# befelix/safe_learning

Measured on NVIDIA H100. Metric: grid-point Lyapunov checks/sec (2D pendulum, M=500 GP), higher is better.
Workload: dtype f64

## Files before the change

### safe_learning_b200/_build.py

```python

from __future__ import annotations

import os
import subprocess
import sys
from concurrent.futures import ThreadPoolExecutor

HERE = os.path.dirname(os.path.abspath(__file__))
CSRC = os.path.join(HERE, "csrc")
OBJDIR = os.path.join(CSRC, "build")
OUTPUT = os.path.join(HERE, "libslb200.so")
HEADER = os.path.join(HERE, "..", "include", "slb200.h")

UNITS = [("gp_tile_%d_%d.o" % (d, tp), "gp_tile_inst.cu", ["-DSLB_TILE_DIN=%d" % d, "-DSLB_TP=%d" % tp],
          ["gp_tile.cuh", "gp_args.h"]) for d in range(1, 7) for tp in (64, 32)]
UNITS += [("gp_sweep.o", "gp_sweep.cu", [], ["gp_args.h"]),
          ("filter.o", "filter.cu", [], ["bulk_copy.cuh", "exp2_tab512.cuh", "gp_mean_staged.cuh", "gp_mean_grid.cuh",
                                         "gp_args.h"]),
          ("light.o", "light.cu", [], ["bulk_copy.cuh", "exp2_tab512.cuh", "gp_mean_staged.cuh", "bellman.cuh"]),
          ("bellman_tile.o", "bellman_tile.cu", [], []),
          ("rollout.o", "rollout.cu", [], ["bulk_copy.cuh", "exp2_tab512.cuh", "gp_mean_staged.cuh", "bellman.cuh"]),
          ("value_opt.o", "value_opt.cu", [], ["bulk_copy.cuh", "exp2_tab512.cuh", "gp_mean_staged.cuh",
                                               "bellman.cuh"]),
          ("network_grad.o", "network_grad.cu", [], []),
          ("triangulation_grad.o", "triangulation_grad.cu", [], []),
          ("gp_grad.o", "gp_grad.cu", [], []),
          ("gp_hyper.o", "gp_hyper.cu", [], []),
          ("no_shrink.o", "no_shrink.cu", [], [])]
SOURCES = sorted({u[1] for u in UNITS})

ARCH = ["-gencode", "arch=compute_90a,code=sm_90a"]
CFLAGS = ARCH + ["-lineinfo", "-O3", "-std=c++17", "-Xcompiler", "-fPIC"]


def _mtime(path):
    return os.path.getmtime(path) if os.path.exists(path) else 0.0


def _unit_stale(unit):
    obj, src, _, headers = unit
    built = _mtime(os.path.join(OBJDIR, obj))
    deps = [os.path.join(CSRC, src), os.path.join(CSRC, "common.cuh"), os.path.join(CSRC, "exp2_tab64.h"),
            HEADER, os.path.abspath(__file__)]
    deps += [os.path.join(CSRC, h) for h in headers]
    return built == 0.0 or any(_mtime(d) > built for d in deps)


def _stale():
    if not os.path.exists(OUTPUT):
        return True
    built = os.path.getmtime(OUTPUT)
    return any(_unit_stale(u) or _mtime(os.path.join(OBJDIR, u[0])) > built for u in UNITS)


def _run(cmd, verbose):
    proc = subprocess.run(cmd, cwd=CSRC, stdout=subprocess.PIPE, stderr=subprocess.STDOUT, text=True)
    if verbose or proc.returncode != 0:
        sys.stderr.write(proc.stdout)
    if proc.returncode != 0:
        raise RuntimeError("nvcc failed (%s):\n%s" % (" ".join(cmd), proc.stdout))
    return proc.stdout


def build_library(force=False, verbose=False, jobs=None):
    if not force and not _stale():
        return OUTPUT
    nvcc = os.environ.get("NVCC", "nvcc")
    os.makedirs(OBJDIR, exist_ok=True)
    todo = [u for u in UNITS if force or _unit_stale(u)]
    extra = ["-Xptxas", "-v"] if verbose else []

    def compile_unit(unit):
        obj, src, flags, _ = unit
        return _run([nvcc] + CFLAGS + extra + flags + ["-c", src, "-o", os.path.join(OBJDIR, obj)],
                    verbose)

    jobs = jobs or min(len(todo) or 1, os.cpu_count() or 1)
    with ThreadPoolExecutor(max_workers=jobs) as pool:
        list(pool.map(compile_unit, todo))
    _run([nvcc, "-shared"] + ARCH + ["-o", OUTPUT] + [os.path.join(OBJDIR, u[0]) for u in UNITS],
         verbose)
    return OUTPUT


if __name__ == "__main__":
    print(build_library(force="--force" in sys.argv, verbose="-v" in sys.argv))
```

### safe_learning_b200/csrc/gp_args.h

```cpp
#pragma once
#include <stdint.h>

enum { MODE_SWEEP_GRID = 0, MODE_SWEEP_STATES = 1, MODE_PREDICT = 2 };
enum { SLB_SPLIT_ITEMS = 512, SLB_SPLIT_MAX = 8, SLB_SPLIT_TICKET_BYTES = 2048 };
#define SLB_SPLIT_PARTIAL_BYTES ((size_t)SLB_SPLIT_ITEMS * SLB_MAX_OUT * (1 + SLB_MAX_OUT) * 64 * sizeof(double))

struct slb_gp_args {
    const double* points;
    int64_t n;
    int64_t idx_begin;
    int32_t mode;
    int32_t want_var;
    uint8_t* negative;
    double* values;
    double* decrease;
    double* threshold;
    double* mean;
    double* err;
    const int64_t* index_list;
    const unsigned long long* count;
    int64_t count_min, count_max;
    double* split_partial;
    int* split_ticket;
    long long* timing;
};

template <int DIN, int TPV>
int slb_gp_tile_launch(cudaStream_t st, const slb_sweep& cfg, const slb_gp_args& a, bool kexpr, bool timing);
```

### safe_learning_b200/csrc/gp_sweep.cu

```cuda
#include "common.cuh"

#include <string.h>

#include "gp_args.h"

namespace {

__global__ void pack_factor_kernel(const double* __restrict__ Linv, int M, int nrb,
                                   double* __restrict__ W, int64_t total) {
    const int64_t e = (int64_t)blockIdx.x * blockDim.x + threadIdx.x;
    if (e >= total) return;
    const int64_t pair = e >> 6;
    const int lane = (int)((e >> 1) & 31);
    const int half = (int)(e & 1);
    int64_t b = (int64_t)((sqrt(8.0 * (double)pair + 1.0) - 1.0) * 0.5);
    while (b * (b + 1) / 2 > pair) --b;
    while ((b + 1) * (b + 2) / 2 <= pair) ++b;
    const int64_t kp = pair - b * (b + 1) / 2;
    const int64_t row = 8 * b + (lane >> 2);
    const int64_t col = 8 * kp + 4 * half + (lane & 3);
    W[e] = (row < M && col <= row) ? Linv[row * M + col] : 0.0;
}


cudaEvent_t g_factor_event[64] = {};
bool g_factor_pending[64] = {};

int wait_for_factors(cudaStream_t st) {
    int device = 0;
    SLB_CUDA(cudaGetDevice(&device));
    if (device < 0 || device >= 64 || !g_factor_pending[device]) return 0;
    cudaStreamCaptureStatus cs = cudaStreamCaptureStatusNone;
    SLB_CUDA(cudaStreamIsCapturing(st, &cs));
    SLB_CUDA(cudaStreamWaitEvent(st, g_factor_event[device],
                                 cs == cudaStreamCaptureStatusActive ? cudaEventWaitExternal : 0));
    return 0;
}

int dispatch_gp_tile(cudaStream_t st, const slb_sweep& cfg, const slb_gp_args& a, int tp = 64) {
    if (a.n <= 0) return 0;
    if (wait_for_factors(st)) return 1;
    SLB_CHECK(a.n <= (int64_t)0x7fffffff * tp, "too many points for one launch");
    const bool timing = a.timing != nullptr;
    bool kexpr = false;
    for (int f = 0; f < cfg.gp.num_factors; ++f) kexpr |= cfg.gp.factors[f].kernel.num_prims > 0;
    return slb_dispatch_dim<1, 6>(cfg.gp.input_dim, "GP input_dim", [&](auto D) {
        return tp == 64 ? slb_gp_tile_launch<D, 64>(st, cfg, a, kexpr, timing)
                        : slb_gp_tile_launch<D, 32>(st, cfg, a, kexpr, timing);
    });
}

}

int slb_wait_for_factors(cudaStream_t st) { return wait_for_factors(st); }

int slb_launch_det_sweep(cudaStream_t st, const slb_sweep& cfg, const double* states, int64_t n,
                         int64_t idx_begin, uint8_t* negative, double* values, double* decrease,
                         double* threshold, double* mean);

static long long* g_timing_buffer = nullptr;

static int64_t g_refine_split = 32 * SLB_NUM_SMS;

int slb_launch_refine(cudaStream_t st, const slb_sweep& cfg, int64_t n_max, int64_t idx_begin,
                      const int64_t* list, const unsigned long long* count, uint8_t* negative,
                      double* values, double* mean, double* err, double* split_partial, int* split_ticket) {
    slb_gp_args a;
    memset(&a, 0, sizeof(a));
    a.idx_begin = idx_begin; a.mode = MODE_SWEEP_GRID;
    a.negative = negative; a.values = values;
    a.mean = mean; a.err = err;
    a.index_list = list; a.count = count;
    a.timing = g_timing_buffer;
    const int tps[2] = {32, 64};
    const int64_t lo[2] = {0, g_refine_split};
    const int64_t hi[2] = {g_refine_split, INT64_MAX};
    for (int v = 0; v < 2; ++v) {
        if (lo[v] >= hi[v] || lo[v] >= n_max) continue;
        a.count_min = lo[v]; a.count_max = hi[v];
        a.n = n_max < hi[v] ? n_max : hi[v];
        a.split_partial = nullptr; a.split_ticket = nullptr;
        if (v == 0 && split_partial != nullptr) {
            if (a.n < (int64_t)SLB_NUM_SMS * tps[v]) a.n = (int64_t)SLB_NUM_SMS * tps[v];
            if ((a.n + tps[v] - 1) / tps[v] <= SLB_SPLIT_ITEMS) {
                a.split_partial = split_partial; a.split_ticket = split_ticket;
            }
        }
        const int rc = dispatch_gp_tile(st, cfg, a, tps[v]);
        if (rc) return rc;
    }
    return 0;
}

extern "C" {

int slb_debug_refine_split(int64_t upto32) {
    g_refine_split = upto32 < 0 ? 0 : upto32;
    return 0;
}

int slb_restore_tables(void* dst_dev, const void* src_host, int64_t split_bytes, int64_t total_bytes,
                       void* stream, void* side_stream) {
    SLB_CHECK(dst_dev != nullptr && src_host != nullptr, "slb_restore_tables: null buffer");
    SLB_CHECK(split_bytes >= 0 && split_bytes <= total_bytes, "slb_restore_tables: split %lld outside [0, %lld]",
              (long long)split_bytes, (long long)total_bytes);
    cudaStream_t st = static_cast<cudaStream_t>(stream), side = static_cast<cudaStream_t>(side_stream);
    char* dst = static_cast<char*>(dst_dev);
    const char* src = static_cast<const char*>(src_host);
    if (split_bytes > 0) SLB_CUDA(cudaMemcpyAsync(dst, src, (size_t)split_bytes, cudaMemcpyHostToDevice, st));
    const int64_t rest = total_bytes - split_bytes;
    if (rest <= 0) return 0;
    if (side == nullptr || side == st) {
        SLB_CUDA(cudaMemcpyAsync(dst + split_bytes, src + split_bytes, (size_t)rest, cudaMemcpyHostToDevice, st));
        return 0;
    }
    int device = 0;
    SLB_CUDA(cudaGetDevice(&device));
    SLB_CHECK(device >= 0 && device < 64, "slb_restore_tables: device %d unsupported", device);
    static cudaEvent_t order[64] = {};
    if (order[device] == nullptr) SLB_CUDA(cudaEventCreateWithFlags(&order[device], cudaEventDisableTiming));
    SLB_CUDA(cudaEventRecord(order[device], st));
    SLB_CUDA(cudaStreamWaitEvent(side, order[device], 0));
    SLB_CUDA(cudaMemcpyAsync(dst + split_bytes, src + split_bytes, (size_t)rest, cudaMemcpyHostToDevice, side));
    return slb_record_factor_dependency(side);
}

int slb_record_factor_dependency(void* stream) {
    int device = 0;
    SLB_CUDA(cudaGetDevice(&device));
    SLB_CHECK(device >= 0 && device < 64, "slb_record_factor_dependency: device %d unsupported", device);
    if (g_factor_event[device] == nullptr)
        SLB_CUDA(cudaEventCreateWithFlags(&g_factor_event[device], cudaEventDisableTiming));
    SLB_CUDA(cudaEventRecord(g_factor_event[device], static_cast<cudaStream_t>(stream)));
    g_factor_pending[device] = true;
    return 0;
}

int slb_debug_phase_timing(void* buffer_dev) {
    g_timing_buffer = static_cast<long long*>(buffer_dev);
    return 0;
}

int64_t slb_packed_len(int32_t M) {
    if (M <= 0) return 0;
    const int64_t nrb = (M + 7) / 8;
    return nrb * (nrb + 1) * 32;
}

int slb_pack_factor(void* stream, const double* Linv_dev, int32_t M, double* Wpack_dev) {
    SLB_CHECK(Linv_dev != nullptr && Wpack_dev != nullptr, "slb_pack_factor: null pointer");
    SLB_CHECK(M > 0, "slb_pack_factor: M must be positive (got %d)", M);
    const int nrb = (M + 7) / 8;
    const int64_t total = slb_packed_len(M);
    const int threads = 256;
    const int64_t blocks = (total + threads - 1) / threads;
    pack_factor_kernel<<<(unsigned)blocks, threads, 0, (cudaStream_t)stream>>>(Linv_dev, M, nrb,
                                                                              Wpack_dev, total);
    SLB_LAUNCH_CHECK();
    return 0;
}

int slb_gp_predict(void* stream, const slb_gp_stack* gp, const double* points_dev, int64_t n,
                   double* mean_dev, double* err_dev, int32_t want_var) {
    SLB_CHECK(gp != nullptr, "slb_gp_predict: null gp");
    if (slb_validate_gp(gp)) return 1;
    SLB_CHECK(gp->num_outputs > 0, "slb_gp_predict: GP stack has no outputs");
    SLB_CHECK(n >= 0, "slb_gp_predict: negative n");
    SLB_CHECK(n == 0 || (points_dev && mean_dev && err_dev), "slb_gp_predict: null buffer");
    slb_sweep cfg;
    memset(&cfg, 0, sizeof(cfg));
    cfg.gp = *gp;
    slb_gp_args a;
    memset(&a, 0, sizeof(a));
    a.points = points_dev; a.n = n; a.mode = MODE_PREDICT; a.want_var = want_var;
    a.mean = mean_dev; a.err = err_dev;
    return dispatch_gp_tile((cudaStream_t)stream, cfg, a);
}

static int sweep_common(void* stream, const slb_sweep* cfg, const double* states, int64_t n,
                        int64_t idx_begin, uint8_t* negative, double* values, double* decrease,
                        double* threshold, double* mean, double* err) {
    int m;
    if (slb_validate_sweep(cfg, states != nullptr, &m)) return 1;
    SLB_CHECK(n >= 0, "lyapunov sweep: negative point count");
    if (n == 0) return 0;
    SLB_CHECK(negative != nullptr, "lyapunov sweep: negative_dev is required");
    if (cfg->gp.num_outputs > 0) {
        slb_gp_args a;
        memset(&a, 0, sizeof(a));
        a.points = states; a.n = n; a.idx_begin = idx_begin;
        a.mode = states ? MODE_SWEEP_STATES : MODE_SWEEP_GRID;
        a.negative = negative; a.values = values; a.decrease = decrease; a.threshold = threshold;
        a.mean = mean; a.err = err;
        a.timing = g_timing_buffer;
        return dispatch_gp_tile((cudaStream_t)stream, *cfg, a);
    }
    SLB_CHECK(err == nullptr, "deterministic dynamics have no error bounds (err_dev must be NULL)");
    return slb_launch_det_sweep((cudaStream_t)stream, *cfg, states, n, idx_begin, negative, values,
                                decrease, threshold, mean);
}

int slb_lyapunov_sweep(void* stream, const slb_sweep* cfg, int64_t idx_begin, int64_t idx_end,
                       uint8_t* negative_dev, double* values_dev, double* decrease_dev,
                       double* threshold_dev, double* mean_dev, double* err_dev) {
    SLB_CHECK(cfg != nullptr, "slb_lyapunov_sweep: null config");
    if (slb_validate_range("slb_lyapunov_sweep", idx_begin, idx_end, cfg->grid.nindex)) return 1;
    return sweep_common(stream, cfg, nullptr, idx_end - idx_begin, idx_begin, negative_dev,
                        values_dev, decrease_dev, threshold_dev, mean_dev, err_dev);
}

int slb_lyapunov_points(void* stream, const slb_sweep* cfg, const double* states_dev, int64_t n,
                        uint8_t* negative_dev, double* values_dev, double* decrease_dev,
                        double* threshold_dev, double* mean_dev, double* err_dev) {
    SLB_CHECK(n == 0 || states_dev != nullptr, "slb_lyapunov_points: null states");
    return sweep_common(stream, cfg, states_dev, n, 0, negative_dev, values_dev, decrease_dev,
                        threshold_dev, mean_dev, err_dev);
}

}
```

### safe_learning_b200/csrc/gp_tile.cuh

```cuda
#pragma once
#define SLB_EVAL_NOINLINE 1
#include "common.cuh"

#include <string.h>

#include <atomic>


#include "gp_args.h"

namespace {

#ifndef SLB_TP
#define SLB_TP SLB_TILE_POINTS
#endif
constexpr int TP = SLB_TP;
static_assert(TP == 32 || TP == 64, "TP must be 32 or 64");
constexpr int PANEL = 256;
constexpr int KSTR = TP + 2;
constexpr int NW = 8;
constexpr int NT = NW * 32;
constexpr int RQ = 32 / NW;
constexpr int NB = TP / 8;
constexpr int CTAS_PER_SM = 1;
constexpr int NRED = 1 + SLB_MAX_OUT;
constexpr int PREFETCH_CTAS = SLB_NUM_SMS * CTAS_PER_SM;

constexpr size_t SMEM_KS = (size_t)(PANEL / 8) * 4 * KSTR * 2 * sizeof(double);
constexpr size_t SMEM_Z = (size_t)SLB_MAX_IN * TP * sizeof(double);
constexpr size_t SMEM_RED = (size_t)NW * TP * NRED * sizeof(double);
constexpr size_t SMEM_TOT = (size_t)NRED * TP * sizeof(double);
constexpr size_t SMEM_POST = (size_t)2 * SLB_MAX_OUT * TP * sizeof(double);
constexpr size_t SMEM_EXPTAB = 64 * sizeof(double);
constexpr size_t SMEM_XP = (size_t)PANEL * SLB_MAX_IN * sizeof(double);
constexpr size_t SMEM_KEXPR = (sizeof(slb_kernel) + 15) / 16 * 16;
constexpr size_t SMEM_PRE = (size_t)4 * TP * sizeof(double);
constexpr size_t SMEM_TOTAL = SMEM_KS + SMEM_Z + SMEM_RED + SMEM_TOT + SMEM_POST + SMEM_EXPTAB +
                              SMEM_XP + SMEM_KEXPR + SMEM_PRE;

SLB_DEV double2 ldg_stream2(const double2* p) {
    double2 v;
    asm volatile("ld.global.nc.L1::no_allocate.v2.f64 {%0, %1}, [%2];"
                 : "=d"(v.x), "=d"(v.y) : "l"(p));
    return v;
}

SLB_DEV void dmma884(double& c0, double& c1, double a, double b) {
    asm volatile("mma.sync.aligned.m8n8k4.row.col.f64.f64.f64.f64 {%0,%1}, {%2}, {%3}, {%0,%1};"
                 : "+d"(c0), "+d"(c1) : "d"(a), "d"(b));
}

constexpr int RING = TP == 64 ? 3 : 5;
constexpr int BG = 4;

template <int Q0>
SLB_DEV void mma_run(double (&acc)[RQ][NB][2], const double2* const (&ap)[RQ], int m0, int m1,
                     const double2* ks_lane) {
    double2 ar[RING][RQ];
    const int m1m = m1 - 1;
#pragma unroll
    for (int d = 0; d < RING; ++d) {
        const int md = min(m0 + d, m1m);
#pragma unroll
        for (int q = Q0; q < RQ; ++q) ar[d][q] = ldg_stream2(ap[q] + md * 32);
    }
    int m = m0;
#pragma unroll 1
    while (true) {
#pragma unroll
        for (int d = 0; d < RING; ++d) {
            if (m >= m1) return;
            const double2* kb = ks_lane + m * (4 * KSTR);
#pragma unroll
            for (int half = 0; half < NB; half += BG) {
                double2 b[BG];
#pragma unroll
                for (int nb = 0; nb < BG; ++nb) b[nb] = kb[(half + nb) * 8];
#pragma unroll
                for (int q = Q0; q < RQ; ++q)
#pragma unroll
                    for (int nb = 0; nb < BG; ++nb)
                        dmma884(acc[q][half + nb][0], acc[q][half + nb][1], ar[d][q].x, b[nb].x);
#pragma unroll
                for (int q = Q0; q < RQ; ++q)
#pragma unroll
                    for (int nb = 0; nb < BG; ++nb)
                        dmma884(acc[q][half + nb][0], acc[q][half + nb][1], ar[d][q].y, b[nb].y);
            }
            const int mp = min(m + RING, m1m);
#pragma unroll
            for (int q = Q0; q < RQ; ++q) ar[d][q] = ldg_stream2(ap[q] + mp * 32);
            ++m;
        }
    }
}

template <int NBT>
SLB_DEV void row_lane_reduce(const double (&v)[2 * NBT], int lane, double* red_q) {
    constexpr int NV = 2 * NBT;
    const bool g2 = (lane & 16) != 0, g1 = (lane & 8) != 0, g0 = (lane & 4) != 0;
    double w8[NV / 2], w4[NV / 4];
#pragma unroll
    for (int i = 0; i < NV / 2; ++i) {
        const double send = g2 ? v[i] : v[i + NV / 2];
        const double keep = g2 ? v[i + NV / 2] : v[i];
        w8[i] = keep + __shfl_xor_sync(0xffffffffu, send, 16);
    }
#pragma unroll
    for (int i = 0; i < NV / 4; ++i) {
        const double send = g1 ? w8[i] : w8[i + NV / 4];
        const double keep = g1 ? w8[i + NV / 4] : w8[i];
        w4[i] = keep + __shfl_xor_sync(0xffffffffu, send, 8);
    }
    if constexpr (NBT == 8) {
        double w2[2];
#pragma unroll
        for (int i = 0; i < 2; ++i) {
            const double send = g0 ? w4[i] : w4[i + 2];
            const double keep = g0 ? w4[i + 2] : w4[i];
            w2[i] = keep + __shfl_xor_sync(0xffffffffu, send, 4);
        }
        double* slot = red_q + (8 * (lane >> 2) + 2 * (lane & 3)) * NRED;
        slot[0] += w2[0];
        slot[NRED] += w2[1];
    } else {
        static_assert(NBT == 4, "written for 8 or 4 column blocks");
        const double send = g0 ? w4[0] : w4[1];
        const double keep = g0 ? w4[1] : w4[0];
        const double w1 = keep + __shfl_xor_sync(0xffffffffu, send, 4);
        const int g = lane >> 2;
        red_q[(8 * (g >> 1) + 2 * (lane & 3) + (g & 1)) * NRED] += w1;
    }
}

template <int DIN, bool TIMING, bool KEXPR>
SLB_DEV void gp_tile_body(const slb_sweep& cfg, const slb_gp_args& a, unsigned char* smem_raw,
                          const int64_t tile_index, const int64_t npts, const int grp, const int G,
                          const int fsel, const int FS, const bool first_tile) {
    double* Ks = reinterpret_cast<double*>(smem_raw);
    double* zraw = Ks + (PANEL / 8) * 4 * KSTR * 2;
    double* red = zraw + SLB_MAX_IN * TP;
    double* tot = red + NW * TP * NRED;
    double* post = tot + NRED * TP;
    double* exptab = post + 2 * SLB_MAX_OUT * TP;
    double* Xp = exptab + 64;
    slb_kernel* kexpr = reinterpret_cast<slb_kernel*>(Xp + PANEL * SLB_MAX_IN);
    double* pre = reinterpret_cast<double*>(reinterpret_cast<unsigned char*>(kexpr) + SMEM_KEXPR);

    const int tid = threadIdx.x, lane = tid & 31, warp = tid >> 5;
    prefetch_descriptor_operands(cfg);
    const double exp_entry = c_exp2_tab[tid & 63];
    const int64_t tile0 = tile_index * TP;
    const int D = cfg.gp.num_outputs;
    long long t_gen = 0, t_mma = 0, t_epi = 0, t_mark = 0, t_sync = 0, t_s0 = 0;
    const long long t_start = TIMING ? clock64() : 0;
    long long g_start = 0;
    if (TIMING) asm volatile("mov.u64 %0, %globaltimer;" : "=l"(g_start));

    if (first_tile && blockIdx.x < PREFETCH_CTAS) {
        for (int f = 0; f < cfg.gp.num_factors; ++f) {
            const slb_gp_factor& F = cfg.gp.factors[f];
            const char* base = reinterpret_cast<const char*>(F.Wpack);
            const size_t nbytes = (size_t)F.nrb * (F.nrb + 1) * 32 * sizeof(double);
            for (size_t off = ((size_t)blockIdx.x * NT + tid) * 128; off < nbytes;
                 off += (size_t)PREFETCH_CTAS * NT * 128)
                asm volatile("prefetch.global.L2 [%0];" ::"l"(base + off));
        }
    }

    if (tid < 64) exptab[tid] = exp_entry;

    if (tid < TP) {
        int64_t rel = tile0 + tid;
        if (rel > npts - 1) rel = npts - 1;
        if (a.index_list != nullptr) rel = a.index_list[rel];
        double z[SLB_MAX_IN];
        if (a.mode == MODE_PREDICT) {
#pragma unroll
            for (int c = 0; c < DIN; ++c) z[c] = a.points[rel * DIN + c];
        } else {
            const int d = cfg.grid.ndim;
            double x[SLB_MAX_DIM];
            if (a.mode == MODE_SWEEP_GRID) {
                grid_index_to_state(cfg.grid, a.idx_begin + rel, x);
            } else {
                for (int c = 0; c < d; ++c) x[c] = a.points[rel * d + c];
            }
            double u[SLB_MAX_OUT];
            const int m = eval_fn_small(cfg.policy, x, u);
            for (int c = 0; c < d; ++c) z[c] = x[c];
            for (int c = 0; c < m; ++c) z[d + c] = u[c];
        }
#pragma unroll
        for (int c = 0; c < DIN; ++c) zraw[c * TP + tid] = z[c];
    } else if (tid < 2 * TP && a.mode != MODE_PREDICT) {
        const int p = tid - TP;
        int64_t rel = tile0 + p;
        if (rel > npts - 1) rel = npts - 1;
        if (a.index_list != nullptr) rel = a.index_list[rel];
        const int d = cfg.grid.ndim;
        double x[SLB_MAX_DIM];
        if (a.mode == MODE_SWEEP_GRID) {
            grid_index_to_state(cfg.grid, a.idx_begin + rel, x);
        } else {
            for (int c = 0; c < d; ++c) x[c] = a.points[rel * d + c];
        }
        lyapunov_state_terms(cfg, x, a.mode == MODE_SWEEP_GRID ? a.idx_begin + rel : -1, &pre[p],
                             &pre[TP + p]);
    }
    __syncthreads();

    const int wg_ = warp & 3, wr_ = warp >> 2;
    const int wslot = wr_ == 0 ? wg_ : 7 - wg_;
    const int p_gen = tid & (TP - 1);
    const int jg = tid / TP;
    const double2* ks_lane = reinterpret_cast<const double2*>(Ks) + (lane & 3) * KSTR + (lane >> 2);

    auto factor_epilogue = [&](int f, bool general, double s2) {
        const slb_gp_factor& F = cfg.gp.factors[f];
        if (tid < TP) {
            int qty = 1;
            for (int o = 0; o < D; ++o) {
                const slb_gp_output& Go = cfg.gp.outputs[o];
                if (Go.factor != f) continue;
                double mx = 0.0;
                if (Go.prior_mean != nullptr) {
                    mx = f64mul(zraw[tid], Go.prior_mean[0]);
                    for (int c = 1; c < DIN; ++c)
                        mx = f64add(mx, f64mul(zraw[c * TP + tid], Go.prior_mean[c]));
                    mx = f64mul(F.scale, mx);
                }
                const double fmean = f64add(tot[qty * TP + tid], mx) / F.scale;
                double kss = F.kss;
                if (general) {
                    double zt[DIN];
#pragma unroll
                    for (int c = 0; c < DIN; ++c) zt[c] = zraw[c * TP + tid];
                    kss = s2 * kernel_expr_diag<DIN>(*kexpr, zt);
                }
                const double fvar = f64sub(kss, tot[tid]) / s2;
                post[o * TP + tid] = fmean;
                post[(SLB_MAX_OUT + o) * TP + tid] =
                    a.want_var ? fvar : f64mul(Go.beta, sqrt(fvar));
                ++qty;
            }
        }
    };

    const bool split = G * FS > 1;
    for (int f = 0; f < cfg.gp.num_factors; ++f) {
        if (fsel >= 0 && f != fsel) continue;
        const slb_gp_factor& F = cfg.gp.factors[f];
        const int M = F.M, nrb = F.nrb;
        const int nk4 = (M + 3) >> 2;
        const double s2 = f64mul(F.scale, F.scale);
        const double variance = F.variance;
        const double* __restrict__ Xs = F.Xs;

        const bool general = KEXPR && F.kernel.num_prims > 0;
        if (general) {
            __syncthreads();
            const int* src = reinterpret_cast<const int*>(&F.kernel);
            for (int i = tid; i < (int)(sizeof(slb_kernel) / sizeof(int)); i += NT)
                reinterpret_cast<int*>(kexpr)[i] = src[i];
            __syncthreads();
        }
        double zs[DIN];
#pragma unroll
        for (int c = 0; c < DIN; ++c)
            zs[c] = general ? zraw[c * TP + p_gen] : zraw[c * TP + p_gen] / F.lengthscales[c];
        for (int i = lane; i < TP * NRED; i += 32) red[warp * TP * NRED + i] = 0.0;
        __syncwarp();
        int resident = -1;

        int rlo = 0, rhi = nrb;
        if (G > 1) {
            rlo = __double2int_rd((double)nrb * sqrt((double)grp / (double)G));
            rhi = grp + 1 == G ? nrb : __double2int_rd((double)nrb * sqrt((double)(grp + 1) / (double)G));
        }
        for (int pbeg = rlo; pbeg < rhi; pbeg += 32) {
            double acc[RQ][NB][2];
#pragma unroll
            for (int q = 0; q < RQ; ++q)
#pragma unroll
                for (int nb = 0; nb < NB; ++nb) { acc[q][nb][0] = 0.0; acc[q][nb][1] = 0.0; }

            const int pend = min(pbeg + 32, rhi);
            int bq[RQ];
#pragma unroll
            for (int q = 0; q < RQ; ++q) bq[q] = pend - 1 - wslot - NW * (RQ - 1 - q);

            const int jp_last = (pend - 1) >> 5;
            for (int jp = 0; jp <= jp_last; ++jp) {
                const int nkp = min(64, nk4 - 64 * jp);
                if (jp != resident) {
                    if (TIMING) t_s0 = clock64();
                    __syncthreads();
                    if (TIMING) { t_mark = clock64(); t_sync += t_mark - t_s0; }
                    const int j0 = PANEL * jp;
                    const int nj = min(PANEL, M - j0);
                    for (int i = tid; i < nj * DIN; i += NT) Xp[i] = Xs[(size_t)j0 * DIN + i];
                    __syncthreads();
                    constexpr int PS = NT / TP / 4;
                    static_assert(NT / TP == 4 * PS, "generation needs a multiple of 4 groups");
                    const int gr = jg & 3, gpo = jg >> 2;
                    const int npairs = (nkp + 1) >> 1;
                    double2* ks2 = reinterpret_cast<double2*>(Ks);
                    constexpr int GP = 2;
                    if (general) {
                        for (int mm = gpo; mm < npairs; mm += GP * PS) {
                            const double* xr[2 * GP];
#pragma unroll
                            for (int u = 0; u < 2 * GP; ++u) {
                                const int jj = 8 * (mm + PS * (u >> 1)) + 4 * (u & 1) + gr;
                                xr[u] = Xp + min(jj, nj - 1) * DIN;
                            }
                            double kv[2 * GP];
                            kernel_expr_cross_n<DIN, 2 * GP>(*kexpr, zs, xr, exptab, kv);
#pragma unroll
                            for (int u = 0; u < 2 * GP; ++u) {
                                const int jj = 8 * (mm + PS * (u >> 1)) + 4 * (u & 1) + gr;
                                kv[u] = jj < nj ? s2 * kv[u] : 0.0;
                            }
#pragma unroll
                            for (int g = 0; g < GP; ++g)
                                if (mm + PS * g < npairs)
                                    ks2[((mm + PS * g) * 4 + gr) * KSTR + p_gen] =
                                        make_double2(kv[2 * g], kv[2 * g + 1]);
                        }
                    } else
                    for (int mm = gpo; mm < npairs; mm += GP * PS) {
                        double t2[2 * GP];
#pragma unroll
                        for (int u = 0; u < 2 * GP; ++u) {
                            const int jj = min(8 * (mm + PS * (u >> 1)) + 4 * (u & 1) + gr, nj - 1);
                            const double* xr = Xp + jj * DIN;
                            double acc2 = 0.0;
#pragma unroll
                            for (int c = 0; c < DIN; ++c) {
                                const double df = zs[c] - xr[c];
                                acc2 = fma(df, df, acc2);
                            }
                            t2[u] = acc2;
                        }
                        double kv[2 * GP];
#pragma unroll
                        for (int u = 0; u < 2 * GP; ++u) {
                            const int jj = 8 * (mm + PS * (u >> 1)) + 4 * (u & 1) + gr;
                            const double k = s2 * (variance * exp_neg_tab(-0.5 * t2[u], exptab));
                            kv[u] = jj < nj ? k : 0.0;
                        }
#pragma unroll
                        for (int g = 0; g < GP; ++g)
                            if (mm + PS * g < npairs)
                                ks2[((mm + PS * g) * 4 + gr) * KSTR + p_gen] =
                                    make_double2(kv[2 * g], kv[2 * g + 1]);
                    }
                    resident = jp;
                    if (TIMING) { t_s0 = clock64(); t_gen += t_s0 - t_mark; }
                    __syncthreads();
                    if (TIMING) t_sync += clock64() - t_s0;
                }
                if (TIMING) t_mark = clock64();
                const int npairs_mma = (nkp + 1) >> 1;
                int mend[RQ];
                const double2* ap[RQ];
#pragma unroll
                for (int q = 0; q < RQ; ++q) {
                    const bool valid = bq[q] >= pbeg;
                    const int me = valid ? min(npairs_mma, max(0, bq[q] - 32 * jp + 1)) : 0;
                    mend[q] = me;
                    const int64_t b = valid ? bq[q] : 0;
                    ap[q] = reinterpret_cast<const double2*>(F.Wpack) +
                            (b * (b + 1) / 2 + 32 * jp) * 32 + lane;
                }
                int mprev = 0;
                if (mend[0] > mprev) { mma_run<0>(acc, ap, mprev, mend[0], ks_lane); mprev = mend[0]; }
                if (mend[1] > mprev) { mma_run<1>(acc, ap, mprev, mend[1], ks_lane); mprev = mend[1]; }
                if (mend[2] > mprev) { mma_run<2>(acc, ap, mprev, mend[2], ks_lane); mprev = mend[2]; }
                if (mend[3] > mprev) { mma_run<3>(acc, ap, mprev, mend[3], ks_lane); mprev = mend[3]; }
                if (TIMING) t_mma += clock64() - t_mark;
            }
            if (TIMING) t_mark = clock64();

            int qty = 0;
            for (int o = -1; o < D; ++o) {
                double al[RQ] = {};
                if (o >= 0) {
                    if (cfg.gp.outputs[o].factor != f) continue;
                    const double* alpha = cfg.gp.outputs[o].alpha;
#pragma unroll
                    for (int q = 0; q < RQ; ++q)
                        if (bq[q] >= pbeg) al[q] = __ldg(alpha + 8 * bq[q] + (lane >> 2));
                }
                constexpr int NV = 2 * NB;
                double v[NV];
#pragma unroll
                for (int nb = 0; nb < NB; ++nb) {
#pragma unroll
                    for (int e = 0; e < 2; ++e) {
                        double t = 0.0;
#pragma unroll
                        for (int q = 0; q < RQ; ++q) {
                            const double x = acc[q][nb][e];
                            t = fma(x, (o < 0) ? x : al[q], t);
                        }
                        v[nb * 2 + e] = t;
                    }
                }
                row_lane_reduce<NB>(v, lane, red + (size_t)warp * TP * NRED + qty);
                ++qty;
            }
            __syncwarp();
            if (TIMING) t_epi += clock64() - t_mark;
        }

        if (TIMING) t_s0 = clock64();
        __syncthreads();
        if (TIMING) t_sync += clock64() - t_s0;
        if (tid < TP) {
            for (int r = 0; r < NRED; ++r) {
                double s = 0.0;
#pragma unroll
                for (int w = 0; w < NW; ++w) s += red[(w * TP + tid) * NRED + r];
                tot[r * TP + tid] = s;
            }
        }
        __syncthreads();

        if (split) {
            double* part = a.split_partial + ((size_t)blockIdx.x * SLB_MAX_OUT + f) * (NRED * TP);
            for (int i = tid; i < NRED * TP; i += NT) part[i] = tot[i];
            __syncthreads();
            continue;
        }
        factor_epilogue(f, general, s2);
        __syncthreads();
    }

    if (split) {
        __shared__ int s_ticket;
        __threadfence();
        __syncthreads();
        if (tid == 0) s_ticket = atomicAdd(a.split_ticket + tile_index, 1);
        __syncthreads();
        if (s_ticket != G * FS - 1) {
            if (TIMING && lane == 0) {
                long long* t = a.timing + ((size_t)blockIdx.x * NW + warp) * 8;
                long long g_end;
                asm volatile("mov.u64 %0, %globaltimer;" : "=l"(g_end));
                t[0] = t_gen; t[1] = t_mma; t[2] = t_epi; t[3] = clock64() - t_start;
                t[4] = g_start; t[5] = g_end; t[6] = t_sync; t[7] = 1;
            }
            return;
        }
        __threadfence();
        if (tid == 0) a.split_ticket[tile_index] = 0;
        for (int f = 0; f < cfg.gp.num_factors; ++f) {
            const slb_gp_factor& F = cfg.gp.factors[f];
            for (int i = tid; i < NRED * TP; i += NT) {
                double sum = 0.0;
                const size_t cta0 = (size_t)tile_index * (G * FS) + (FS > 1 ? (size_t)f * G : 0);
                for (int g2 = 0; g2 < G; ++g2)
                    sum += __ldcg(a.split_partial + ((cta0 + g2) * SLB_MAX_OUT + f) * (NRED * TP) + i);
                tot[i] = sum;
            }
            const bool general = KEXPR && F.kernel.num_prims > 0;
            if (general) {
                const int* src = reinterpret_cast<const int*>(&F.kernel);
                for (int i = tid; i < (int)(sizeof(slb_kernel) / sizeof(int)); i += NT)
                    reinterpret_cast<int*>(kexpr)[i] = src[i];
            }
            __syncthreads();
            factor_epilogue(f, general, f64mul(F.scale, F.scale));
            __syncthreads();
        }
    }

    if (TIMING && lane == 0) {
        long long* t = a.timing + ((size_t)blockIdx.x * NW + warp) * 8;
        long long g_end;
        asm volatile("mov.u64 %0, %globaltimer;" : "=l"(g_end));
        t[0] = t_gen; t[1] = t_mma; t[2] = t_epi; t[3] = clock64() - t_start;
        t[4] = g_start; t[5] = g_end; t[6] = t_sync; t[7] = 0;
    }
    {
        const int p = tid & (TP - 1);
        const bool live = tile0 + p < npts;
        int64_t rel = live ? tile0 + p : 0;
        if (a.index_list != nullptr) rel = a.index_list[rel];
        if (tid < 2 * TP && live) {
            double mu[SLB_MAX_OUT], er[SLB_MAX_OUT];
            for (int o = 0; o < D; ++o) {
                mu[o] = post[o * TP + p];
                er[o] = post[(SLB_MAX_OUT + o) * TP + p];
            }
            if (tid < TP) {
                if (a.mean != nullptr) for (int o = 0; o < D; ++o) a.mean[rel * D + o] = mu[o];
                if (a.err != nullptr) for (int o = 0; o < D; ++o) a.err[rel * D + o] = er[o];
                if (a.mode != MODE_PREDICT) {
                    double vm[1];
                    eval_fn_small(cfg.lyapunov, mu, vm);
                    pre[2 * TP + p] = vm[0];
                }
            } else if (a.mode != MODE_PREDICT) {
                pre[3 * TP + p] = lyapunov_error_bound(cfg, mu, er);
            }
        }
        if (a.mode == MODE_PREDICT) return;
        __syncthreads();
        if (tid < TP && live) {
            const slb_decision r =
                lyapunov_combine(pre[p], pre[TP + p], pre[2 * TP + p], pre[3 * TP + p]);
            a.negative[rel] = r.negative ? 1 : 0;
            if (a.values != nullptr) a.values[rel] = r.vx;
            if (a.decrease != nullptr) a.decrease[rel] = r.decrease;
            if (a.threshold != nullptr) a.threshold[rel] = r.threshold;
        }
    }
}

template <int DIN, bool TIMING, bool KEXPR, int TPV>
__global__ void __launch_bounds__(NT, CTAS_PER_SM)
gp_tile_kernel(const __grid_constant__ slb_sweep cfg, const slb_gp_args a) {
    extern __shared__ __align__(16) unsigned char smem_raw[];
    int64_t tile_index = blockIdx.x;
    int64_t tile_end = tile_index + 1, tile_step = 1;
    int grp = 0, G = 1;
    int fsel = -1, FS = 1;
    int64_t npts = a.n;
    if (a.count != nullptr) {
        prefetch_descriptor_operands(cfg);
        npts = (int64_t)*a.count;
        if (npts <= a.count_min || npts > a.count_max) return;
        const int64_t ntiles = (npts + TP - 1) / TP;
        if (a.split_partial != nullptr) {
            int64_t spare = (int64_t)gridDim.x / ntiles;
            const int nfac = cfg.gp.num_factors;
            if (nfac > 1 && spare >= 2 * nfac) {
                FS = nfac;
                spare /= nfac;
            }
            G = (int)(spare < 1 ? 1 : (spare > SLB_SPLIT_MAX ? SLB_SPLIT_MAX : spare));
            const int per_tile = G * FS;
            if ((int64_t)blockIdx.x >= ntiles * per_tile) return;
            tile_index = blockIdx.x / per_tile;
            tile_end = tile_index + 1;
            const int rem = (int)(blockIdx.x % per_tile);
            grp = rem % G;
            if (FS > 1) fsel = rem / G;
        } else {
            tile_end = ntiles;
            tile_step = gridDim.x;
        }
        if (tile_index * TP >= npts) return;
    }
    for (int64_t tile = tile_index; tile < tile_end; tile += tile_step) {
        gp_tile_body<DIN, TIMING, KEXPR>(cfg, a, smem_raw, tile, npts, grp, G, fsel, FS, tile == tile_index);
        if (tile + tile_step < tile_end) __syncthreads();
    }
}

template <int DIN, bool TIMING, bool KEXPR, int TPV = TP>
int launch_gp_tile(cudaStream_t st, const slb_sweep& cfg, const slb_gp_args& a) {
    static_assert(TPV == TP, "TPV only disambiguates the symbol");
    static std::atomic<bool> configured[64];
    int device = 0;
    SLB_CUDA(cudaGetDevice(&device));
    if (device < 0 || device >= 64 || !configured[device].load(std::memory_order_acquire)) {
        SLB_CUDA(cudaFuncSetAttribute(gp_tile_kernel<DIN, TIMING, KEXPR, TP>,
                                      cudaFuncAttributeMaxDynamicSharedMemorySize,
                                      (int)SMEM_TOTAL));
        if (device >= 0 && device < 64) configured[device].store(true, std::memory_order_release);
    }
    int64_t tiles = (a.n + TP - 1) / TP;
    if (a.count != nullptr && a.split_partial == nullptr && tiles > PREFETCH_CTAS) tiles = PREFETCH_CTAS;
    gp_tile_kernel<DIN, TIMING, KEXPR, TP><<<(unsigned)tiles, NT, SMEM_TOTAL, st>>>(cfg, a);
    SLB_LAUNCH_CHECK();
    return 0;
}

}
```

### safe_learning_b200/csrc/gp_tile_inst.cu

```cuda
#include "gp_tile.cuh"

#ifndef SLB_TILE_DIN
#error "compile with -DSLB_TILE_DIN=<1..6>"
#endif

template <int DIN, int TPV>
int slb_gp_tile_launch(cudaStream_t st, const slb_sweep& cfg, const slb_gp_args& a, bool kexpr,
                       bool timing) {
#if SLB_TILE_DIN == 3 && SLB_TP == 64
    if (timing) return launch_gp_tile<3, true, false>(st, cfg, a);
#else
    if (timing) {
        slb_set_error("phase timing is compiled for d_in = 3, 64-point tiles only");
        return 1;
    }
#endif
    return kexpr ? launch_gp_tile<DIN, false, true>(st, cfg, a)
                 : launch_gp_tile<DIN, false, false>(st, cfg, a);
}

template int slb_gp_tile_launch<SLB_TILE_DIN, SLB_TP>(cudaStream_t, const slb_sweep&, const slb_gp_args&,
                                                      bool, bool);
```

Before: 546.9 million.

## Merge two refine launches into one kernel choosing tile size on device

The refine path used to launch two GP tile kernels, a 32-point variant and a 64-point variant, each gated by count ranges. Now one refine kernel reads the device-side count and branches between the 32-point split path and the 64-point persistent path, with the long path in a noinline function. This removes one kernel launch per refine and the empty launch that used to exit early. The sweep kernel is simplified to a plain per-tile launch, and the timing instrumentation is extended. The change adds register pressure and code-size risk from putting both tile sizes in one kernel.

```diff
diff --git a/safe_learning_b200/_build.py b/safe_learning_b200/_build.py
--- a/safe_learning_b200/_build.py
+++ b/safe_learning_b200/_build.py
@@ -12,8 +12,8 @@
 OUTPUT = os.path.join(HERE, "libslb200.so")
 HEADER = os.path.join(HERE, "..", "include", "slb200.h")
 
-UNITS = [("gp_tile_%d_%d.o" % (d, tp), "gp_tile_inst.cu", ["-DSLB_TILE_DIN=%d" % d, "-DSLB_TP=%d" % tp],
-          ["gp_tile.cuh", "gp_args.h"]) for d in range(1, 7) for tp in (64, 32)]
+UNITS = [("gp_%s_%d.o" % (kind, d), "gp_tile_inst.cu", ["-DSLB_TILE_DIN=%d" % d, "-DSLB_REFINE=%d" % refine],
+          ["gp_tile.cuh", "gp_args.h"]) for d in range(1, 7) for kind, refine in (("tile", 0), ("refine", 1))]
 UNITS += [("gp_sweep.o", "gp_sweep.cu", [], ["gp_args.h"]),
           ("filter.o", "filter.cu", [], ["bulk_copy.cuh", "exp2_tab512.cuh", "gp_mean_staged.cuh", "gp_mean_grid.cuh",
                                          "gp_args.h"]),
diff --git a/safe_learning_b200/csrc/gp_args.h b/safe_learning_b200/csrc/gp_args.h
--- a/safe_learning_b200/csrc/gp_args.h
+++ b/safe_learning_b200/csrc/gp_args.h
@@ -19,11 +19,13 @@
     double* err;
     const int64_t* index_list;
     const unsigned long long* count;
-    int64_t count_min, count_max;
+    int64_t split_max;
     double* split_partial;
     int* split_ticket;
     long long* timing;
 };
 
-template <int DIN, int TPV>
+template <int DIN>
 int slb_gp_tile_launch(cudaStream_t st, const slb_sweep& cfg, const slb_gp_args& a, bool kexpr, bool timing);
+template <int DIN>
+int slb_gp_refine_launch(cudaStream_t st, const slb_sweep& cfg, const slb_gp_args& a, bool kexpr, bool timing);
diff --git a/safe_learning_b200/csrc/gp_sweep.cu b/safe_learning_b200/csrc/gp_sweep.cu
--- a/safe_learning_b200/csrc/gp_sweep.cu
+++ b/safe_learning_b200/csrc/gp_sweep.cu
@@ -37,16 +37,16 @@
     return 0;
 }
 
-int dispatch_gp_tile(cudaStream_t st, const slb_sweep& cfg, const slb_gp_args& a, int tp = 64) {
+int dispatch_gp_tile(cudaStream_t st, const slb_sweep& cfg, const slb_gp_args& a, bool refine = false) {
     if (a.n <= 0) return 0;
     if (wait_for_factors(st)) return 1;
-    SLB_CHECK(a.n <= (int64_t)0x7fffffff * tp, "too many points for one launch");
+    SLB_CHECK(a.n <= (int64_t)0x7fffffff * 64, "too many points for one launch");
     const bool timing = a.timing != nullptr;
     bool kexpr = false;
     for (int f = 0; f < cfg.gp.num_factors; ++f) kexpr |= cfg.gp.factors[f].kernel.num_prims > 0;
     return slb_dispatch_dim<1, 6>(cfg.gp.input_dim, "GP input_dim", [&](auto D) {
-        return tp == 64 ? slb_gp_tile_launch<D, 64>(st, cfg, a, kexpr, timing)
-                        : slb_gp_tile_launch<D, 32>(st, cfg, a, kexpr, timing);
+        return refine ? slb_gp_refine_launch<D>(st, cfg, a, kexpr, timing)
+                      : slb_gp_tile_launch<D>(st, cfg, a, kexpr, timing);
     });
 }
 
@@ -65,31 +65,20 @@
 int slb_launch_refine(cudaStream_t st, const slb_sweep& cfg, int64_t n_max, int64_t idx_begin,
                       const int64_t* list, const unsigned long long* count, uint8_t* negative,
                       double* values, double* mean, double* err, double* split_partial, int* split_ticket) {
+    static_assert(SLB_NUM_SMS <= SLB_SPLIT_ITEMS, "the split workspace holds one wave of refine CTAs");
     slb_gp_args a;
     memset(&a, 0, sizeof(a));
-    a.idx_begin = idx_begin; a.mode = MODE_SWEEP_GRID;
+    a.n = n_max; a.idx_begin = idx_begin; a.mode = MODE_SWEEP_GRID;
     a.negative = negative; a.values = values;
     a.mean = mean; a.err = err;
     a.index_list = list; a.count = count;
+    a.split_max = g_refine_split;
     a.timing = g_timing_buffer;
-    const int tps[2] = {32, 64};
-    const int64_t lo[2] = {0, g_refine_split};
-    const int64_t hi[2] = {g_refine_split, INT64_MAX};
-    for (int v = 0; v < 2; ++v) {
-        if (lo[v] >= hi[v] || lo[v] >= n_max) continue;
-        a.count_min = lo[v]; a.count_max = hi[v];
-        a.n = n_max < hi[v] ? n_max : hi[v];
-        a.split_partial = nullptr; a.split_ticket = nullptr;
-        if (v == 0 && split_partial != nullptr) {
-            if (a.n < (int64_t)SLB_NUM_SMS * tps[v]) a.n = (int64_t)SLB_NUM_SMS * tps[v];
-            if ((a.n + tps[v] - 1) / tps[v] <= SLB_SPLIT_ITEMS) {
-                a.split_partial = split_partial; a.split_ticket = split_ticket;
-            }
-        }
-        const int rc = dispatch_gp_tile(st, cfg, a, tps[v]);
-        if (rc) return rc;
+    const int64_t upto32 = n_max < g_refine_split ? n_max : g_refine_split;
+    if (split_partial != nullptr && upto32 <= (int64_t)SLB_SPLIT_ITEMS * 32) {
+        a.split_partial = split_partial; a.split_ticket = split_ticket;
     }
-    return 0;
+    return dispatch_gp_tile(st, cfg, a, true);
 }
 
 extern "C" {
diff --git a/safe_learning_b200/csrc/gp_tile.cuh b/safe_learning_b200/csrc/gp_tile.cuh
--- a/safe_learning_b200/csrc/gp_tile.cuh
+++ b/safe_learning_b200/csrc/gp_tile.cuh
@@ -11,32 +11,22 @@
 
 namespace {
 
-#ifndef SLB_TP
-#define SLB_TP SLB_TILE_POINTS
-#endif
-constexpr int TP = SLB_TP;
-static_assert(TP == 32 || TP == 64, "TP must be 32 or 64");
 constexpr int PANEL = 256;
-constexpr int KSTR = TP + 2;
+template <int TP> constexpr int kstr_of = TP + 2;
 constexpr int NW = 8;
 constexpr int NT = NW * 32;
 constexpr int RQ = 32 / NW;
-constexpr int NB = TP / 8;
 constexpr int CTAS_PER_SM = 1;
 constexpr int NRED = 1 + SLB_MAX_OUT;
 constexpr int PREFETCH_CTAS = SLB_NUM_SMS * CTAS_PER_SM;
 
-constexpr size_t SMEM_KS = (size_t)(PANEL / 8) * 4 * KSTR * 2 * sizeof(double);
-constexpr size_t SMEM_Z = (size_t)SLB_MAX_IN * TP * sizeof(double);
-constexpr size_t SMEM_RED = (size_t)NW * TP * NRED * sizeof(double);
-constexpr size_t SMEM_TOT = (size_t)NRED * TP * sizeof(double);
-constexpr size_t SMEM_POST = (size_t)2 * SLB_MAX_OUT * TP * sizeof(double);
-constexpr size_t SMEM_EXPTAB = 64 * sizeof(double);
-constexpr size_t SMEM_XP = (size_t)PANEL * SLB_MAX_IN * sizeof(double);
 constexpr size_t SMEM_KEXPR = (sizeof(slb_kernel) + 15) / 16 * 16;
-constexpr size_t SMEM_PRE = (size_t)4 * TP * sizeof(double);
-constexpr size_t SMEM_TOTAL = SMEM_KS + SMEM_Z + SMEM_RED + SMEM_TOT + SMEM_POST + SMEM_EXPTAB +
-                              SMEM_XP + SMEM_KEXPR + SMEM_PRE;
+constexpr size_t smem_total(int TP) {
+    return (size_t)(PANEL / 8) * 4 * (TP + 2) * 2 * sizeof(double) + (size_t)SLB_MAX_IN * TP * sizeof(double) +
+           (size_t)NW * TP * NRED * sizeof(double) + (size_t)NRED * TP * sizeof(double) +
+           (size_t)2 * SLB_MAX_OUT * TP * sizeof(double) + 64 * sizeof(double) +
+           (size_t)PANEL * SLB_MAX_IN * sizeof(double) + SMEM_KEXPR + (size_t)4 * TP * sizeof(double);
+}
 
 SLB_DEV double2 ldg_stream2(const double2* p) {
     double2 v;
@@ -45,17 +35,24 @@
     return v;
 }
 
+SLB_DEV long long globaltimer() {
+    long long t;
+    asm volatile("mov.u64 %0, %globaltimer;" : "=l"(t));
+    return t;
+}
+
 SLB_DEV void dmma884(double& c0, double& c1, double a, double b) {
     asm volatile("mma.sync.aligned.m8n8k4.row.col.f64.f64.f64.f64 {%0,%1}, {%2}, {%3}, {%0,%1};"
                  : "+d"(c0), "+d"(c1) : "d"(a), "d"(b));
 }
 
-constexpr int RING = TP == 64 ? 3 : 5;
+template <int TP> constexpr int ring_of = TP == 64 ? 3 : 5;
 constexpr int BG = 4;
 
-template <int Q0>
+template <int Q0, int TP, int NB = TP / 8>
 SLB_DEV void mma_run(double (&acc)[RQ][NB][2], const double2* const (&ap)[RQ], int m0, int m1,
                      const double2* ks_lane) {
+    constexpr int RING = ring_of<TP>, KSTR = kstr_of<TP>;
     double2 ar[RING][RQ];
     const int m1m = m1 - 1;
 #pragma unroll
@@ -133,10 +130,12 @@
     }
 }
 
-template <int DIN, bool TIMING, bool KEXPR>
+template <int DIN, bool TIMING, bool KEXPR, int TP>
 SLB_DEV void gp_tile_body(const slb_sweep& cfg, const slb_gp_args& a, unsigned char* smem_raw,
                           const int64_t tile_index, const int64_t npts, const int grp, const int G,
                           const int fsel, const int FS, const bool first_tile) {
+    static_assert(TP == 32 || TP == 64, "TP must be 32 or 64");
+    constexpr int KSTR = kstr_of<TP>, NB = TP / 8;
     double* Ks = reinterpret_cast<double*>(smem_raw);
     double* zraw = Ks + (PANEL / 8) * 4 * KSTR * 2;
     double* red = zraw + SLB_MAX_IN * TP;
@@ -154,8 +153,17 @@
     const int D = cfg.gp.num_outputs;
     long long t_gen = 0, t_mma = 0, t_epi = 0, t_mark = 0, t_sync = 0, t_s0 = 0;
     const long long t_start = TIMING ? clock64() : 0;
-    long long g_start = 0;
-    if (TIMING) asm volatile("mov.u64 %0, %globaltimer;" : "=l"(g_start));
+    long long g_start = 0, g_gen = 0, g_mma = 0, g_part = 0, g_ticket = 0, g_fin = 0;
+    if (TIMING) g_start = globaltimer();
+    auto write_timing = [&](bool finisher) {
+        if (!TIMING || lane != 0) return;
+        long long* t = a.timing + ((size_t)blockIdx.x * NW + warp) * 16;
+        const long long g_end = globaltimer();
+        t[0] = t_gen; t[1] = t_mma; t[2] = t_epi; t[3] = clock64() - t_start;
+        t[4] = g_start; t[5] = g_end; t[6] = t_sync; t[7] = 0;
+        t[8] = g_start; t[9] = g_gen; t[10] = g_mma; t[11] = g_part;
+        t[12] = g_ticket; t[13] = g_fin; t[14] = g_end; t[15] = finisher ? 1 : 0;
+    };
 
     if (first_tile && blockIdx.x < PREFETCH_CTAS) {
         for (int f = 0; f < cfg.gp.num_factors; ++f) {
@@ -357,7 +365,7 @@
                                     make_double2(kv[2 * g], kv[2 * g + 1]);
                     }
                     resident = jp;
-                    if (TIMING) { t_s0 = clock64(); t_gen += t_s0 - t_mark; }
+                    if (TIMING) { t_s0 = clock64(); t_gen += t_s0 - t_mark; g_gen = globaltimer(); }
                     __syncthreads();
                     if (TIMING) t_sync += clock64() - t_s0;
                 }
@@ -375,11 +383,11 @@
                             (b * (b + 1) / 2 + 32 * jp) * 32 + lane;
                 }
                 int mprev = 0;
-                if (mend[0] > mprev) { mma_run<0>(acc, ap, mprev, mend[0], ks_lane); mprev = mend[0]; }
-                if (mend[1] > mprev) { mma_run<1>(acc, ap, mprev, mend[1], ks_lane); mprev = mend[1]; }
-                if (mend[2] > mprev) { mma_run<2>(acc, ap, mprev, mend[2], ks_lane); mprev = mend[2]; }
-                if (mend[3] > mprev) { mma_run<3>(acc, ap, mprev, mend[3], ks_lane); mprev = mend[3]; }
-                if (TIMING) t_mma += clock64() - t_mark;
+                if (mend[0] > mprev) { mma_run<0, TP>(acc, ap, mprev, mend[0], ks_lane); mprev = mend[0]; }
+                if (mend[1] > mprev) { mma_run<1, TP>(acc, ap, mprev, mend[1], ks_lane); mprev = mend[1]; }
+                if (mend[2] > mprev) { mma_run<2, TP>(acc, ap, mprev, mend[2], ks_lane); mprev = mend[2]; }
+                if (mend[3] > mprev) { mma_run<3, TP>(acc, ap, mprev, mend[3], ks_lane); mprev = mend[3]; }
+                if (TIMING) { t_mma += clock64() - t_mark; g_mma = globaltimer(); }
             }
             if (TIMING) t_mark = clock64();
 
@@ -432,6 +440,7 @@
             double* part = a.split_partial + ((size_t)blockIdx.x * SLB_MAX_OUT + f) * (NRED * TP);
             for (int i = tid; i < NRED * TP; i += NT) part[i] = tot[i];
             __syncthreads();
+            if (TIMING) g_part = globaltimer();
             continue;
         }
         factor_epilogue(f, general, s2);
@@ -444,14 +453,9 @@
         __syncthreads();
         if (tid == 0) s_ticket = atomicAdd(a.split_ticket + tile_index, 1);
         __syncthreads();
+        if (TIMING) g_ticket = globaltimer();
         if (s_ticket != G * FS - 1) {
-            if (TIMING && lane == 0) {
-                long long* t = a.timing + ((size_t)blockIdx.x * NW + warp) * 8;
-                long long g_end;
-                asm volatile("mov.u64 %0, %globaltimer;" : "=l"(g_end));
-                t[0] = t_gen; t[1] = t_mma; t[2] = t_epi; t[3] = clock64() - t_start;
-                t[4] = g_start; t[5] = g_end; t[6] = t_sync; t[7] = 1;
-            }
+            write_timing(false);
             return;
         }
         __threadfence();
@@ -477,13 +481,7 @@
         }
     }
 
-    if (TIMING && lane == 0) {
-        long long* t = a.timing + ((size_t)blockIdx.x * NW + warp) * 8;
-        long long g_end;
-        asm volatile("mov.u64 %0, %globaltimer;" : "=l"(g_end));
-        t[0] = t_gen; t[1] = t_mma; t[2] = t_epi; t[3] = clock64() - t_start;
-        t[4] = g_start; t[5] = g_end; t[6] = t_sync; t[7] = 0;
-    }
+    if (TIMING) g_fin = globaltimer();
     {
         const int p = tid & (TP - 1);
         const bool live = tile0 + p < npts;
@@ -507,7 +505,7 @@
                 pre[3 * TP + p] = lyapunov_error_bound(cfg, mu, er);
             }
         }
-        if (a.mode == MODE_PREDICT) return;
+        if (a.mode == MODE_PREDICT) { write_timing(true); return; }
         __syncthreads();
         if (tid < TP && live) {
             const slb_decision r =
@@ -518,66 +516,93 @@
             if (a.threshold != nullptr) a.threshold[rel] = r.threshold;
         }
     }
-}
-
-template <int DIN, bool TIMING, bool KEXPR, int TPV>
-__global__ void __launch_bounds__(NT, CTAS_PER_SM)
-gp_tile_kernel(const __grid_constant__ slb_sweep cfg, const slb_gp_args a) {
-    extern __shared__ __align__(16) unsigned char smem_raw[];
+    write_timing(true);
+}
+
+template <int DIN, bool TIMING, bool KEXPR, int TP>
+SLB_DEV void refine_tiles(const slb_sweep& cfg, const slb_gp_args& a, unsigned char* smem_raw, int64_t npts) {
     int64_t tile_index = blockIdx.x;
     int64_t tile_end = tile_index + 1, tile_step = 1;
     int grp = 0, G = 1;
     int fsel = -1, FS = 1;
-    int64_t npts = a.n;
-    if (a.count != nullptr) {
-        prefetch_descriptor_operands(cfg);
-        npts = (int64_t)*a.count;
-        if (npts <= a.count_min || npts > a.count_max) return;
-        const int64_t ntiles = (npts + TP - 1) / TP;
-        if (a.split_partial != nullptr) {
-            int64_t spare = (int64_t)gridDim.x / ntiles;
-            const int nfac = cfg.gp.num_factors;
-            if (nfac > 1 && spare >= 2 * nfac) {
-                FS = nfac;
-                spare /= nfac;
-            }
-            G = (int)(spare < 1 ? 1 : (spare > SLB_SPLIT_MAX ? SLB_SPLIT_MAX : spare));
-            const int per_tile = G * FS;
-            if ((int64_t)blockIdx.x >= ntiles * per_tile) return;
-            tile_index = blockIdx.x / per_tile;
-            tile_end = tile_index + 1;
-            const int rem = (int)(blockIdx.x % per_tile);
-            grp = rem % G;
-            if (FS > 1) fsel = rem / G;
-        } else {
-            tile_end = ntiles;
-            tile_step = gridDim.x;
-        }
-        if (tile_index * TP >= npts) return;
+    const int64_t ntiles = (npts + TP - 1) / TP;
+    if (TP == 32 && a.split_partial != nullptr && ntiles <= (int64_t)gridDim.x) {
+        int64_t spare = (int64_t)gridDim.x / ntiles;
+        const int nfac = cfg.gp.num_factors;
+        if (nfac > 1 && spare >= 2 * nfac) {
+            FS = nfac;
+            spare /= nfac;
+        }
+        G = (int)(spare > SLB_SPLIT_MAX ? SLB_SPLIT_MAX : spare);
+        const int per_tile = G * FS;
+        if ((int64_t)blockIdx.x >= ntiles * per_tile) return;
+        tile_index = blockIdx.x / per_tile;
+        tile_end = tile_index + 1;
+        const int rem = (int)(blockIdx.x % per_tile);
+        grp = rem % G;
+        if (FS > 1) fsel = rem / G;
+    } else {
+        tile_end = ntiles;
+        tile_step = gridDim.x;
     }
     for (int64_t tile = tile_index; tile < tile_end; tile += tile_step) {
-        gp_tile_body<DIN, TIMING, KEXPR>(cfg, a, smem_raw, tile, npts, grp, G, fsel, FS, tile == tile_index);
+        gp_tile_body<DIN, TIMING, KEXPR, TP>(cfg, a, smem_raw, tile, npts, grp, G, fsel, FS, tile == tile_index);
         if (tile + tile_step < tile_end) __syncthreads();
     }
 }
 
-template <int DIN, bool TIMING, bool KEXPR, int TPV = TP>
-int launch_gp_tile(cudaStream_t st, const slb_sweep& cfg, const slb_gp_args& a) {
-    static_assert(TPV == TP, "TPV only disambiguates the symbol");
-    static std::atomic<bool> configured[64];
+template <int DIN, bool TIMING, bool KEXPR>
+__device__ __noinline__ void refine_long(const slb_sweep& cfg, const slb_gp_args& a, unsigned char* smem_raw,
+                                         int64_t npts) {
+    refine_tiles<DIN, TIMING, KEXPR, 64>(cfg, a, smem_raw, npts);
+}
+
+template <int DIN, bool TIMING, bool KEXPR>
+__global__ void __launch_bounds__(NT, CTAS_PER_SM)
+gp_tile_kernel(const __grid_constant__ slb_sweep cfg, const slb_gp_args a) {
+    extern __shared__ __align__(16) unsigned char smem_raw[];
+    gp_tile_body<DIN, TIMING, KEXPR, 64>(cfg, a, smem_raw, blockIdx.x, a.n, 0, 1, -1, 1, true);
+}
+
+template <int DIN, bool TIMING, bool KEXPR>
+__global__ void __launch_bounds__(NT, CTAS_PER_SM)
+gp_refine_kernel(const __grid_constant__ slb_sweep cfg, const slb_gp_args a) {
+    extern __shared__ __align__(16) unsigned char smem_raw[];
+    prefetch_descriptor_operands(cfg);
+    const int64_t npts = (int64_t)*a.count;
+    if (npts == 0) return;
+    if (npts <= a.split_max) refine_tiles<DIN, TIMING, KEXPR, 32>(cfg, a, smem_raw, npts);
+    else refine_long<DIN, TIMING, KEXPR>(cfg, a, smem_raw, npts);
+}
+
+template <typename Kernel>
+int configure_smem(Kernel kernel, std::atomic<bool> (&configured)[64]) {
     int device = 0;
     SLB_CUDA(cudaGetDevice(&device));
     if (device < 0 || device >= 64 || !configured[device].load(std::memory_order_acquire)) {
-        SLB_CUDA(cudaFuncSetAttribute(gp_tile_kernel<DIN, TIMING, KEXPR, TP>,
-                                      cudaFuncAttributeMaxDynamicSharedMemorySize,
-                                      (int)SMEM_TOTAL));
+        SLB_CUDA(cudaFuncSetAttribute(kernel, cudaFuncAttributeMaxDynamicSharedMemorySize, (int)smem_total(64)));
         if (device >= 0 && device < 64) configured[device].store(true, std::memory_order_release);
     }
-    int64_t tiles = (a.n + TP - 1) / TP;
-    if (a.count != nullptr && a.split_partial == nullptr && tiles > PREFETCH_CTAS) tiles = PREFETCH_CTAS;
-    gp_tile_kernel<DIN, TIMING, KEXPR, TP><<<(unsigned)tiles, NT, SMEM_TOTAL, st>>>(cfg, a);
+    return 0;
+}
+
+template <int DIN, bool TIMING, bool KEXPR>
+int launch_gp_tile(cudaStream_t st, const slb_sweep& cfg, const slb_gp_args& a) {
+    static std::atomic<bool> configured[64];
+    if (configure_smem(gp_tile_kernel<DIN, TIMING, KEXPR>, configured)) return 1;
+    const int64_t tiles = (a.n + 63) / 64;
+    gp_tile_kernel<DIN, TIMING, KEXPR><<<(unsigned)tiles, NT, smem_total(64), st>>>(cfg, a);
     SLB_LAUNCH_CHECK();
     return 0;
 }
 
-}
+template <int DIN, bool TIMING, bool KEXPR>
+int launch_gp_refine(cudaStream_t st, const slb_sweep& cfg, const slb_gp_args& a) {
+    static std::atomic<bool> configured[64];
+    if (configure_smem(gp_refine_kernel<DIN, TIMING, KEXPR>, configured)) return 1;
+    gp_refine_kernel<DIN, TIMING, KEXPR><<<PREFETCH_CTAS, NT, smem_total(64), st>>>(cfg, a);
+    SLB_LAUNCH_CHECK();
+    return 0;
+}
+
+}
diff --git a/safe_learning_b200/csrc/gp_tile_inst.cu b/safe_learning_b200/csrc/gp_tile_inst.cu
--- a/safe_learning_b200/csrc/gp_tile_inst.cu
+++ b/safe_learning_b200/csrc/gp_tile_inst.cu
@@ -4,14 +4,30 @@
 #error "compile with -DSLB_TILE_DIN=<1..6>"
 #endif
 
-template <int DIN, int TPV>
-int slb_gp_tile_launch(cudaStream_t st, const slb_sweep& cfg, const slb_gp_args& a, bool kexpr,
-                       bool timing) {
-#if SLB_TILE_DIN == 3 && SLB_TP == 64
+#if SLB_REFINE
+template <int DIN>
+int slb_gp_refine_launch(cudaStream_t st, const slb_sweep& cfg, const slb_gp_args& a, bool kexpr, bool timing) {
+#if SLB_TILE_DIN == 3
+    if (timing) return launch_gp_refine<3, true, false>(st, cfg, a);
+#else
+    if (timing) {
+        slb_set_error("phase timing is compiled for d_in = 3 only");
+        return 1;
+    }
+#endif
+    return kexpr ? launch_gp_refine<DIN, false, true>(st, cfg, a)
+                 : launch_gp_refine<DIN, false, false>(st, cfg, a);
+}
+
+template int slb_gp_refine_launch<SLB_TILE_DIN>(cudaStream_t, const slb_sweep&, const slb_gp_args&, bool, bool);
+#else
+template <int DIN>
+int slb_gp_tile_launch(cudaStream_t st, const slb_sweep& cfg, const slb_gp_args& a, bool kexpr, bool timing) {
+#if SLB_TILE_DIN == 3
     if (timing) return launch_gp_tile<3, true, false>(st, cfg, a);
 #else
     if (timing) {
-        slb_set_error("phase timing is compiled for d_in = 3, 64-point tiles only");
+        slb_set_error("phase timing is compiled for d_in = 3 only");
         return 1;
     }
 #endif
@@ -19,5 +35,5 @@
                  : launch_gp_tile<DIN, false, false>(st, cfg, a);
 }
 
-template int slb_gp_tile_launch<SLB_TILE_DIN, SLB_TP>(cudaStream_t, const slb_sweep&, const slb_gp_args&,
-                                                      bool, bool);
+template int slb_gp_tile_launch<SLB_TILE_DIN>(cudaStream_t, const slb_sweep&, const slb_gp_args&, bool, bool);
+#endif
```

After: 551.4 million (median of 6 runs). About the same (+0.8%).
